# burlachenkok/flpytorch

Hardware: AMD Instinct MI355X
Metric: gradient-codec encode+reduce GB/s (device-resident), [N,D] fp32; % HBM peak (higher is better)
Workload: dtype f32; 1 GPU; C3 topk:1% N=1024/GPU D=10000000; codec=topk:1%, clients_per_gpu=1024, clients_total=1024, D=10000000, K=100000, rows_alloc=contiguous, parallelism=client-shard dp1

## Files before the change

flpytorch_amd/_lib.py:

```python
import collections
import ctypes
import os
import threading

_HERE = os.path.dirname(os.path.abspath(__file__))
VARIANT_DIR = os.path.join(os.path.dirname(_HERE), "abvar")
LIB_PATH = (os.path.join(VARIANT_DIR, "libflcodec_%s.so" % os.environ["FLC_LIB_VARIANT"])
            if os.environ.get("FLC_LIB_VARIANT") else os.path.join(_HERE, "libflcodec.so"))

FLC_OK, FLC_ERR_ARG, FLC_ERR_DTYPE, FLC_ERR_HIP, FLC_ERR_WORKSPACE, FLC_ERR_UNSUPPORTED = range(6)
FLC_IDENT, FLC_LAZY, FLC_RANDK, FLC_NATURAL, FLC_STD_DITHERING, FLC_NAT_DITHERING, FLC_TOPK, FLC_RANK_K = range(1, 9)
FLC_NORM_LINF, FLC_NORM_L1, FLC_NORM_L2 = 0, 1, 2
FLC_REDUCE_PLAIN, FLC_REDUCE_REL_X = 0, 1
FLC_PATH_AUTO, FLC_PATH_SPARSE, FLC_PATH_DENSE = 0, 1, 2
FLC_TIE_LOWEST, FLC_TIE_HIGHEST = 0, 1
FLC_NORMMODE_EXACT, FLC_NORMMODE_TORCH_CPU = 0, 1
ABI_VERSION = 104


def FLC_ROW_GROUPS(g):
    return (int(g) & 0xFF) << 8

EXPORTS = [
    "flc_version", "flc_build_id", "flc_last_error_string",
    "flc_reduce_rows", "flc_reduce_matrix",
    "flc_encode_workspace_size", "flc_encode",
    "flc_encode_reduce_workspace_size", "flc_encode_reduce",
    "flc_encode_reduce_ex_workspace_size", "flc_encode_reduce_ex",
    "flc_encode_shift_workspace_size", "flc_encode_shift",
    "flc_encode_shift_reduce_workspace_size", "flc_encode_shift_reduce",
    "flc_randk_shift_reduce_workspace_size", "flc_randk_shift_reduce",
    "flc_topk_shift_reduce_workspace_size", "flc_topk_shift_reduce",
    "flc_dither_shift_reduce_workspace_size", "flc_dither_shift_reduce", "flc_dither_row_flags",
    "flc_payload_bytes", "flc_payload_format", "flc_payload_validate", "flc_pack_workspace_size", "flc_pack", "flc_unpack",
    "flc_unpack_reduce_workspace_size", "flc_unpack_reduce",
    "flc_pack_shift_workspace_size", "flc_pack_shift",
    "flc_unpack_shift_reduce_workspace_size", "flc_unpack_shift_reduce",
    "flc_combine_workspace_size", "flc_combine_partials",
    "flc_combine_blocks_workspace_size", "flc_combine_blocks",
    "flc_mt_choice", "flc_mt_rand", "flc_mt_randint31",
    "flc_device_uniform", "flc_device_randk_indices",
    "flc_device_randk_counts_workspace_size", "flc_device_randk_counts",
    "flc_profile_enable", "flc_profile_collect", "flc_select_row_flags",
    "flc_selftest_division", "flc_norm2_torch_cpu", "flc_debug_resident",
    "flc_norm2_torch_cpu_workspace_size", "flc_norm2_torch_cpu_ws", "flc_rows_alloc", "flc_rows_free",
]


class FlcCodecParams(ctypes.Structure):
    _fields_ = [
        ("codec", ctypes.c_int32),
        ("s", ctypes.c_int32),
        ("norm", ctypes.c_int32),
        ("flags", ctypes.c_int32),
        ("k", ctypes.c_int64),
        ("lazy_p", ctypes.c_float),
        ("randk_scale", ctypes.c_float),
        ("d_levels", ctypes.c_void_p),
        ("seed", ctypes.c_uint64),
        ("tie", ctypes.c_int32),
    ]


class FlcPattern(ctypes.Structure):
    _fields_ = [
        ("d_randk_idx", ctypes.c_void_p),
        ("d_uniforms", ctypes.c_void_p),
        ("d_lazy_u", ctypes.c_void_p),
        ("client0", ctypes.c_int64),
        ("uniforms_ld", ctypes.c_int64),
        ("idx_ld", ctypes.c_int64),
        ("d_randk_counts", ctypes.c_void_p),
    ]


class FlcShiftRows(ctypes.Structure):
    _fields_ = [
        ("d_a", ctypes.c_void_p), ("lda", ctypes.c_int64),
# ... 127 lines not shown
                                       vp, sz, vp]
        lib.flc_unpack_shift_reduce_workspace_size.argtypes = [P(FlcCodecParams), i64, i64]
        lib.flc_unpack_shift_reduce_workspace_size.restype = sz
        lib.flc_unpack_shift_reduce.argtypes = [P(FlcCodecParams), P(FlcPayloadRows), i64, i64, vp, f32, vp, vp, sz, vp]
    lib.flc_combine_workspace_size.argtypes = [vp, i64, i32]
    lib.flc_combine_workspace_size.restype = sz
    lib.flc_combine_partials.argtypes = [vp, vp, i64, f32, i32, vp, sz, vp]
    lib.flc_combine_blocks_workspace_size.argtypes = [vp, i64, i64]
    lib.flc_combine_blocks_workspace_size.restype = sz
    lib.flc_combine_blocks.argtypes = [vp, vp, i64, i64, i64, f32, vp, vp, sz, vp]
    lib.flc_mt_choice.argtypes = [vp, vp, i64, i64, vp, vp]
    lib.flc_mt_rand.argtypes = [vp, vp, i64, vp]
    lib.flc_mt_randint31.argtypes = [vp, vp, i64, vp]
    lib.flc_device_uniform.argtypes = [ctypes.c_uint64, i64, i64]
    lib.flc_device_uniform.restype = ctypes.c_double
    lib.flc_device_randk_indices.argtypes = [ctypes.c_uint64, i64, i64, i64, vp]
    lib.flc_device_randk_counts_workspace_size.argtypes = [i64, i64]
    lib.flc_device_randk_counts_workspace_size.restype = sz
    lib.flc_device_randk_counts.argtypes = [ctypes.c_uint64, i64, i64, i64, i64, vp, vp, sz, vp]
    lib.flc_profile_enable.argtypes = [i32]
    lib.flc_profile_collect.argtypes = [ctypes.c_char_p, vp, vp]
    lib.flc_selftest_division.argtypes = [vp, i32, vp, vp]
    if hasattr(lib, "flc_norm2_torch_cpu"):
        lib.flc_norm2_torch_cpu.argtypes = [vp, i64, i64, i64, vp, vp]
    if hasattr(lib, "flc_norm2_torch_cpu_ws"):
        lib.flc_norm2_torch_cpu_workspace_size.argtypes = [i64, i64]
        lib.flc_norm2_torch_cpu_workspace_size.restype = sz
        lib.flc_norm2_torch_cpu_ws.argtypes = [vp, i64, i64, i64, vp, vp, sz, vp]
    if hasattr(lib, "flc_rows_alloc"):
        lib.flc_rows_alloc.argtypes = [sz, i32, vp]
        lib.flc_rows_free.argtypes = [vp]
    if hasattr(lib, "flc_debug_resident"):
        lib.flc_debug_resident.argtypes = [i32, i64]
    if hasattr(lib, "flc_select_row_flags"):
        lib.flc_select_row_flags.argtypes = [P(FlcCodecParams), i64, i64, vp, sz, vp, vp]
    for name in EXPORTS:
        if not hasattr(lib, name):
            continue
        if name not in ("flc_version", "flc_build_id", "flc_last_error_string", "flc_device_uniform",
                        "flc_encode_workspace_size", "flc_encode_reduce_workspace_size",
                        "flc_encode_reduce_ex_workspace_size", "flc_encode_shift_workspace_size",
                        "flc_encode_shift_reduce_workspace_size", "flc_randk_shift_reduce_workspace_size",
                        "flc_topk_shift_reduce_workspace_size", "flc_dither_shift_reduce_workspace_size",
                        "flc_payload_bytes", "flc_pack_workspace_size",
                        "flc_pack_shift_workspace_size", "flc_unpack_shift_reduce_workspace_size",
                        "flc_unpack_reduce_workspace_size", "flc_combine_workspace_size",
                        "flc_combine_blocks_workspace_size", "flc_device_randk_counts_workspace_size",
                        "flc_norm2_torch_cpu_workspace_size"):
            getattr(lib, name).restype = i32
    return lib


def source_hash(root=None):
    import glob
    import hashlib
    root = root or os.path.dirname(_HERE)
    csrc = os.path.join(root, "flpytorch_amd", "csrc")
    files = sorted(glob.glob(os.path.join(csrc, "*.hip")) + glob.glob(os.path.join(csrc, "*.hpp")) +
                   glob.glob(os.path.join(csrc, "*.cpp")))
    files += [os.path.join(csrc, "Makefile"), os.path.join(root, "include", "flcodec.h")]
    h = hashlib.sha256()
    for f in files:
        with open(f, "rb") as fh:
            h.update(fh.read())
    return h.hexdigest()[:16]

# ... 89 lines not shown
```

flpytorch_amd/csrc/api.hip:

```cpp
#include <stdarg.h>
#include <stdio.h>

#include <algorithm>
#include <map>
#include <mutex>
#include <string>
#include <vector>

#include "common.hpp"

namespace flc {

static thread_local char g_err[512] = "";

void set_error(const char* fmt, ...) {
    va_list ap;
    va_start(ap, fmt);
    vsnprintf(g_err, sizeof(g_err), fmt, ap);
    va_end(ap);
}

int hip_fail(hipError_t e, const char* what) {
    set_error("%s: %s", what, hipGetErrorString(e));
    return FLC_ERR_HIP;
// ... 155 lines not shown
    if (!d_ptr || bytes == 0) { set_error("flc_rows_alloc: bad args"); return FLC_ERR_ARG; }
    *d_ptr = nullptr;
    const hipError_t e = contiguous ? hipExtMallocWithFlags(d_ptr, bytes, hipDeviceMallocContiguous) : hipMalloc(d_ptr, bytes);
    if (e != hipSuccess) {
        (void)hipGetLastError();
        *d_ptr = nullptr;
        set_error("flc_rows_alloc: %s of %zu bytes failed: %s", contiguous ? "contiguous allocation" : "hipMalloc", bytes,
                  hipGetErrorString(e));
        return FLC_ERR_HIP;
    }
    return FLC_OK;
}

extern "C" int flc_rows_free(void* d_ptr) {
    if (d_ptr && hipFree(d_ptr) != hipSuccess) { set_error("flc_rows_free: hipFree failed"); return FLC_ERR_HIP; }
    return FLC_OK;
}

extern "C" size_t flc_norm2_torch_cpu_workspace_size(int64_t n, int64_t d) {
    return (n <= 0 || d < 0) ? 0 : norm_torch_ws_bytes(n, d);
}

extern "C" int flc_norm2_torch_cpu_ws(const float* d_rows, int64_t ld, int64_t n, int64_t d, float* d_out, void* d_ws,
                                      size_t ws_bytes, void* stream) {
    if (n < 0 || d < 0 || (n > 1 && ld < d) || (n > 0 && (!d_rows || !d_out || !d_ws))) {
        set_error("flc_norm2_torch_cpu_ws: bad args (n=%lld d=%lld ld=%lld)", (long long)n, (long long)d, (long long)ld);
        return FLC_ERR_ARG;
    }
    if (n == 0) return FLC_OK;
    return norm_torch_ws_run(d_rows, ld, n, d, d_out, d_ws, ws_bytes, (hipStream_t)stream);
}

extern "C" int flc_debug_resident(int grid_mult, int64_t spin_ticks) { return rs_debug(grid_mult, spin_ticks); }

extern "C" int flc_norm2_torch_cpu(const float* d_rows, int64_t ld, int64_t n, int64_t d, float* d_out, void* stream) {
    if (n < 0 || d < 0 || (n > 1 && ld < d) || (n > 0 && (!d_rows || !d_out))) {
        set_error("flc_norm2_torch_cpu: bad args (n=%lld d=%lld ld=%lld)", (long long)n, (long long)d, (long long)ld);
        return FLC_ERR_ARG;
    }
    if (n == 0) return FLC_OK;
    return norm_torch_run(d_rows, ld, n, d, d_out, (hipStream_t)stream);
}

namespace flc {
int selftest_division(const float* d_b, int nb, unsigned long long* d_bad, hipStream_t st);
}
extern "C" int flc_selftest_division(const float* d_divisors, int n, unsigned long long* d_mismatches,
                                     void* stream) {
    if (n < 0 || (n > 0 && (!d_divisors || !d_mismatches))) { set_error("flc_selftest_division: bad args"); return FLC_ERR_ARG; }
    if (n == 0) return FLC_OK;
    return selftest_division(d_divisors, n, d_mismatches, (hipStream_t)stream);
}

namespace flc {
size_t encode_row_workspace(const flc_codec_params* prm, int64_t d) {
    if (prm->codec == FLC_TOPK) return sel_workspace(prm, 1, d);
    if (prm->codec == FLC_RANK_K) return rk_workspace(prm, 1, d, false);
    if (prm->codec == FLC_RANDK) return randk_device_workspace(1, d);
    return ew_workspace(prm, 1, d);
}
}

extern "C" size_t flc_encode_workspace_size(const flc_codec_params* prm, int64_t d) {
    if (!prm || !known(prm->codec)) return 0;
    if (prm->codec == FLC_TOPK) return sel_workspace(prm, 1, d);
    if (prm->codec == FLC_RANK_K) return rk_workspace(prm, 1, d, false);
// ... 348 lines not shown
```

flpytorch_amd/csrc/chunk_accum.hip:

```cpp
#include "select_impl.hpp"

namespace flc {

constexpr int AP = FLC_CA_AP;

struct RowMeta {
    uint2 te;
    uint32_t thr, cut, mode;
    float w;
};

__device__ inline RowMeta load_meta(const SelWs& ws, int64_t c, int64_t n, int64_t r, const float* w, int64_t rend = -1) {
    RowMeta m;
    m.te = make_uint2(0, 0);
    m.thr = 0; m.cut = 0u; m.mode = 0; m.w = 1.f;
    if (r < (rend < 0 ? n : rend)) {
        m.te = ws.tab[c * n + r];
        m.thr = ws.thr[r];
        const uint32_t f = ws.flags[r];
        m.mode = (f & F_EXACT) ? 2u : ((f & F_TIES) ? 1u : 0u);
        if (m.mode == 1u) m.cut = tie_pref(ws.tiecut[r], ws.tie_hi);
        if (m.mode == 2u) m.thr = 0u;
        if (w) m.w = w[r];
    }
// ... 81 lines not shown
        if (w && (__float_as_uint(w[r]) >> 31)) continue;
#pragma unroll
        for (int j = 0; j < WL; ++j) if (lane + 64 * j < NW) rm[lane + 64 * j] = 0u;
        __threadfence_block();
        const RowMeta m = load_meta(ws, c, n, r, w);
        const uint32_t mode = m.mode, T = m.thr, cut = m.cut;
        for (uint32_t e = (uint32_t)lane; e < m.te.y; e += 64) {
            const uint32_t ix = ws.ent_idx[r * ws.cap + m.te.x + e];
            const uint32_t key = mag_key(ws.ent_val[r * ws.cap + m.te.x + e]);
            const uint32_t loc = ix - cbase;
            if (loc < (uint32_t)TS && (mode == 2u || key > T || (key == T && tie_pref(ix, ws.tie_hi) >= cut)))
                atomicOr(&rm[loc >> 5], 1u << (loc & 31));
        }
        __threadfence_block();
        bool left = false;
#pragma unroll
        for (int j = 0; j < WL; ++j) {
            if (lane + 64 * j < NW) zc[j] &= atomicOr(&rm[lane + 64 * j], 0u);
            left |= zc[j] != 0u;
        }
        if (__ballot(left) == 0ull) break;
    }
#pragma unroll
    for (int j = 0; j < WL; ++j) {
        uint32_t dead = z0[j] & ~zc[j];
        while (dead) {
            const int b = __builtin_ctz(dead);
            dead &= dead - 1u;
            tl[(lane + 64 * j) * 32 + b] = 0.f;
        }
    }
}

template <bool ASSIGN, int TS, bool W, int WPB, int AP = AP>
__device__ __forceinline__ void chunk_accum_body(int64_t n, int64_t d, SelWs ws, const float* __restrict__ w, float wt,
                                                 float* __restrict__ out, int64_t r0, int64_t rend, int first, int last,
                                                 float (*tile)[TS], uint32_t (*zmask)[WPB == 1 ? 1 : TS / 32]) {
    if (rend < 0) rend = n;
    constexpr int PARTS = CHUNK / TS;
    const int lane = threadIdx.x & 63;
    const int wv = WPB == 1 ? 0 : __builtin_amdgcn_readfirstlane(threadIdx.x >> 6);
    const int64_t C = nchunks(d);
    float* tl = tile[wv];
    const int64_t nb = (rend - r0 + 63) / 64;
    for (int64_t t = (int64_t)blockIdx.x * WPB + wv; t < C * PARTS; t += (int64_t)gridDim.x * WPB) {
        const int64_t c = t / PARTS;
        const uint32_t cbase = (uint32_t)(c * CHUNK + (t % PARTS) * TS);
        if (FLC_TILE_V4 && !ASSIGN && !first && (int64_t)cbase + TS <= d) {
            const float4* p4 = reinterpret_cast<const float4*>(ws.part + cbase);
#pragma unroll
            for (int k0 = 0; k0 < TS / 256; k0 += 8) {
                float4 v[8];
#pragma unroll
                for (int k = 0; k < 8; ++k) v[k] = k0 + k < TS / 256 ? p4[(k0 + k) * 64 + lane] : make_float4(0.f, 0.f, 0.f, 0.f);
#pragma unroll
                for (int k = 0; k < 8; ++k)
                    if (k0 + k < TS / 256) reinterpret_cast<float4*>(tl)[(k0 + k) * 64 + lane] = v[k];
            }
        } else {
            for (int i = lane; i < TS; i += 64)
                tl[i] = ASSIGN ? 0.f : (first || (int64_t)cbase + i >= d ? -0.f : ws.part[cbase + i]);
        }
        RowMeta cur = load_meta(ws, c, n, r0 + lane, w, rend), nxt;
        uint32_t ri[AP][2];
        float rv[AP][2];
        auto fetch = [&](const RowMeta& m, int q, int64_t row, int slot) {
            const uint32_t off = __builtin_amdgcn_readlane(m.te.x, q), cnt = __builtin_amdgcn_readlane(m.te.y, q);
            const auto di = list_rsrc(ws.ent_idx + row * ws.cap + off, cnt);
            const auto dv = list_rsrc(ws.ent_val + row * ws.cap + off, cnt);
#pragma unroll
            for (int h = 0; h < 2; ++h) {
                const uint32_t e = (uint32_t)lane + 64u * h;
                const uint32_t x = __builtin_amdgcn_raw_buffer_load_b32(di, lane * 4, h * 256, 0);
                ri[slot][h] = e < cnt ? x : 0xFFFFFFFFu;
                rv[slot][h] = __uint_as_float(__builtin_amdgcn_raw_buffer_load_b32(dv, lane * 4, h * 256, 0));
            }
        };
        const uint32_t txm = ws.tie_hi ? 0u : 0xFFFFFFFFu;
// ... 62 lines not shown
                    for (int z = 0; z < AP; ++z)
                        if (z == slot) { ri[z][0] = xi[0]; ri[z][1] = xi[1]; rv[z][0] = xv[0]; rv[z][1] = xv[1]; }
                }
            }
            cur = nxt;
        }
        const int64_t len = min((int64_t)TS, d - (int64_t)cbase);
        if (!last) {
            for (int64_t i = lane; i < len; i += 64) ws.part[cbase + i] = tl[i];
            continue;
        }
        if (!ASSIGN) {
            if (WPB == 1) resolve_neg_zero_g<TS>(tl, ws.zm + t * (TS / 32), ws, c, n, cbase, len, w, lane);
            else resolve_neg_zero<TS>(tl, zmask[wv], ws, c, n, cbase, len, w, lane);
        }
        for (int64_t i = lane; i < len; i += 64) out[cbase + i] = ASSIGN ? tl[i] : tl[i] / wt;
    }
}

template <bool ASSIGN, int TS = CHUNK, bool W = true>
__global__ __launch_bounds__(256) void k_chunk_accum(int64_t n, int64_t d, SelWs ws, const float* __restrict__ w, float wt,
                                                     float* __restrict__ out, int64_t r0 = 0, int64_t rend = -1,
                                                     int first = 1, int last = 1) {
    __shared__ __attribute__((aligned(16))) float tile[4][TS];
    __shared__ uint32_t zmask[4][TS / 32];
    chunk_accum_body<ASSIGN, TS, W, 4>(n, d, ws, w, wt, out, r0, rend, first, last, tile, zmask);
}

template <bool W>
__global__ __launch_bounds__(64) void k_chunk_accum1(
        int64_t n, int64_t d, SelWs ws, const float* __restrict__ w, float wt, float* __restrict__ out, int64_t r0,
        int64_t rend, int first, int last) {
    extern __shared__ __attribute__((aligned(16))) float dyn_tile[];
    chunk_accum_body<false, CHUNK, W, 1, FLC_CA_AP1>(n, d, ws, w, wt, out, r0, rend, first, last,
                                         reinterpret_cast<float (*)[CHUNK]>(dyn_tile), nullptr);
}

__global__ __launch_bounds__(256) void k_assign_scatter(SelWs ws, float* __restrict__ out, int sharded) {
    const uint32_t T = ws.thr[0], f = ws.flags[0];
    const uint32_t mode = (f & F_EXACT) ? 2u : ((f & F_TIES) ? 1u : 0u);
    const uint32_t cut = mode == 1u ? tie_pref(ws.tiecut[0], ws.tie_hi) : 0u;
    const bool shd = sharded && mode != 2u;
    const int64_t segcap = (ws.cap / CS_SH) & ~int64_t(3);
    for (int sh = shd ? (int)blockIdx.x : 0; sh < (shd ? CS_SH : 1); sh += shd ? (int)gridDim.x : 1) {
        const uint32_t cnt = shd ? ws.shcnt[sh * RCS] : ws.rowcnt[0];
        const int64_t o = shd ? sh * segcap : 0;
        for (uint32_t e = (shd ? 0u : blockIdx.x * 256u) + threadIdx.x; e < cnt; e += shd ? 256u : gridDim.x * 256u) {
            const uint32_t ix = ws.ent_idx[o + e];
            const float v = ws.ent_val[o + e];
            const uint32_t key = mag_key(v);
            if (mode == 2u || key > T || (key == T && tie_pref(ix, ws.tie_hi) >= cut)) out[ix] = v;
        }
    }
}

static int accum_parts() {
    static const int p = [] {
        const char* e = tuning_env("FLC_ACCUM_PARTS");
        const int v = e ? atoi(e) : 0;
        return (v == 1 || v == 2 || v == 4) ? v : 0;
    }();
    return p;
}

int launch_group_fold(int64_t n, int64_t d, SelWs ws, const float* w, float wt, float* out, int64_t r0, int64_t r1,
                      bool first, bool last, bool exposed, hipStream_t st) {
    const int64_t C = host_chunks(d);
// ... 57 lines not shown
```

flpytorch_amd/csrc/common.hpp:

```cpp
#pragma once
#include <hip/hip_runtime.h>
#include <stdint.h>
#include <stdlib.h>
#include <string.h>

#include "../../include/flcodec.h"

namespace flc {

constexpr int WAVE = 64;
constexpr int CHUNK = 4096;
constexpr int CHUNK_SHIFT = 12;

void set_error(const char* fmt, ...);
int hip_fail(hipError_t e, const char* what);

#define FLC_CHECK_HIP(expr)                                          \
    do {                                                             \
        hipError_t _e = (expr);                                      \
        if (_e != hipSuccess) return ::flc::hip_fail(_e, #expr);     \
    } while (0)
#define FLC_CHECK_LAUNCH(what)                                       \
    do {                                                             \
        hipError_t _e = hipGetLastError();                           \
// ... 129 lines not shown
int shift_epi_launch(const float* e, int64_t d, const ShiftArgs& sh, hipStream_t st);
int shift_fold_launch(const float* m, int64_t d, const float* w, int64_t i, bool last, float wt, float* acc,
                      hipStream_t st);
enum { SHAPE_D = 0, SHAPE_A = 1, SHAPE_C = 2, SHAPE_B = 3 };
int shift_shape(const flc_shift_rows& sr, const char* me);
int inplace_rows_check(const char* me, int shape, const flc_shift_rows& sr, int64_t n, int64_t d);
int sparse_round_precheck(const char* me, int shape, const flc_shift_rows& sr, int64_t n, int64_t d, int64_t K);
int fold_updated_rows(const flc_shift_rows& sr, int64_t n, int64_t d, const float* w, float wt, float* out, hipStream_t st);
int64_t pack_blocks(int64_t d);
int pack_sparse_launch(const float* dense, int64_t d, int64_t cap, uint32_t* bc, char* payload, hipStream_t st);
size_t pack_shift_workspace(const flc_codec_params* prm, int64_t d);
int pack_shift_run(const flc_codec_params* prm, const flc_pattern* pat, const float* a, int64_t d, const ShiftArgs& sh,
                   char* payload, void* ws, size_t ws_bytes, hipStream_t st);
size_t unpack_shift_reduce_workspace(const flc_codec_params* prm, int64_t n, int64_t d);
int unpack_shift_reduce_run(const flc_codec_params* prm, const flc_payload_rows& pr, int64_t n, int64_t d,
                            const float* w, float wt, float* out, void* ws, size_t ws_bytes, hipStream_t st);
inline int64_t group_row(int64_t n, int G, int g, int lastpct) {
    lastpct = lastpct < 1 ? 1 : lastpct;
    if (G <= 1 || lastpct >= 100) return n * g / G;
    const int64_t unit = 100 * (int64_t)(G - 1) + lastpct;
    const int64_t cum = g <= G - 1 ? 100 * (int64_t)g : unit;
    return n * cum / unit;
}
int norm_torch_run(const float* x, int64_t ld, int64_t n, int64_t d, float* out, hipStream_t st);
size_t norm_torch_ws_bytes(int64_t n, int64_t d);
int norm_torch_ws_run(const float* x, int64_t ld, int64_t n, int64_t d, float* out, void* wsp, size_t ws_bytes,
                      hipStream_t st);
int tn_run(RowSrc rows, int64_t n, int64_t r0, int64_t rn, int64_t d, float* out, void* wsp, const double* item_sums,
           int64_t G, hipStream_t st);
size_t sel_workspace(const flc_codec_params* prm, int64_t n, int64_t d);
int sel_run(const flc_codec_params* prm, const flc_pattern* pat, RowSrc rows, bool vec, int64_t n, int64_t d,
            bool assign, const float* w, float wt, float* out, void* wsp, size_t ws_bytes, hipStream_t st);
int rs_debug(int mult, int64_t spin_ticks);
int sel_row_flags(const flc_codec_params* prm, int64_t n, int64_t d, const void* wsp, size_t ws_bytes,
                  uint32_t* flags, hipStream_t st);
bool ds_eligible(const flc_codec_params* prm, const flc_pattern* pat, int64_t n, int64_t d);
size_t ds_workspace(const flc_codec_params* prm, int64_t n, int64_t d, int norm_mode = FLC_NORMMODE_EXACT);
int ds_run(const flc_codec_params* prm, const flc_pattern* pat, RowSrc rows, int64_t n, int64_t d, const float* w,
           float wt, float* pnorm_out, float* out, void* wsp, size_t ws_bytes, hipStream_t st,
           const float* pnorm_in = nullptr, int norm_mode = FLC_NORMMODE_EXACT);
size_t rk_workspace(const flc_codec_params* prm, int64_t n, int64_t d, bool reduce);
int rk_run(const flc_codec_params* prm, RowSrc rows, int64_t n, int64_t d, bool reduce, const float* w, float wt,
           float* out, void* wsp, size_t ws_bytes, hipStream_t st);
size_t randk_device_workspace(int64_t n, int64_t d);
int randk_device_counts(uint64_t seed, int64_t client0, int64_t n, int64_t d, int64_t k, uint32_t* cnt, void* ws,
                        size_t ws_bytes, hipStream_t st);
int randk_device_prepare(const flc_codec_params* prm, const flc_pattern* pat, int64_t n, int64_t d, void* wsp,
                         const uint32_t** cnt, const uint64_t** ckey, hipStream_t st);
struct RkLists {
    const uint2* tab;
    const uint32_t* idx;
    float* val;
    int64_t cap;
};
size_t randk_lists_workspace(int64_t n, int64_t d, int64_t K);
int randk_lists_build(const flc_codec_params* prm, const flc_pattern* pat, RowSrc rows, int64_t n, int64_t d, void* wsp,
                      RkLists* lists, hipStream_t st);
int randk_lists_fold(int64_t n, int64_t d, int64_t K, void* wsp, const float* w, float wt, float* out, hipStream_t st);
size_t randk_shift_workspace(const flc_codec_params* prm, bool compat, int64_t n, int64_t d);
int randk_shift_run(const flc_codec_params* prm, const flc_pattern* pat, const flc_shift_rows& sr, int64_t n, int64_t d,
                    const float* w, float wt, float* out, void* ws, size_t ws_bytes, hipStream_t st);
int randk_shift_lfold_launch(const float* base, int64_t n, int64_t d, RkLists lists, const float* w, float wt, float* out,
                             hipStream_t st);
constexpr uint32_t TK_F_TIES = 4u, TK_F_EXACT = 8u;
struct TkLists {
    const uint2* tab;
// ... 111 lines not shown
```

flpytorch_amd/csrc/select.hip:

```cpp
#include "select_impl.hpp"

namespace flc {

int64_t sel_capacity(int codec, int64_t d, int64_t K) {
    if (codec == FLC_RANDK) return std::max<int64_t>(K, 1);
    int64_t cap = 2 * K + 2 * CHUNK;
    cap = std::min<int64_t>(std::max<int64_t>(cap, 1), std::max<int64_t>(d, 1));
    return (cap + 3) & ~int64_t(3);
}

SelWs carve_sel(void* base, int codec, int64_t n, int64_t d, int64_t K, size_t* bytes) {
    Carver cv(base);
    const int64_t C = std::max<int64_t>(host_chunks(d), 1), nn = std::max<int64_t>(n, 1);
    SelWs s;
    s.tie_hi = 0;
    s.cap = sel_capacity(codec, d, K);
    s.tab = cv.take<uint2>((size_t)C * nn);
    s.ent_idx = cv.take<uint32_t>((size_t)nn * s.cap);
    s.ent_val = cv.take<float>((size_t)nn * s.cap);
    s.rowcnt = cv.take<uint32_t>((size_t)nn * RCS);
    s.flags = cv.take<uint32_t>(nn);
    s.thr = cv.take<uint32_t>(nn);
    s.prefix = cv.take<uint32_t>(nn);
    s.krem = cv.take<uint32_t>(nn);
// ... 74 lines not shown

static int topk_fast_groups(const TkCall& c) {
    const int64_t n = c.n, d = c.d;
    const SelWs& ws = c.ws;
    const hipStream_t st = c.st;
    const bool few = c.few;
    const int TG = few ? 1 : tk_tail_groups(c.prm, n);
    hipStream_t sside = st;
    TkCtx* cx = nullptr;
    std::unique_lock<std::mutex> lk;
    if (TG > 1) {
        int dev = 0;
        FLC_CHECK_HIP(hipGetDevice(&dev));
        lk = std::unique_lock<std::mutex>(g_tk_mu);
        cx = &g_tk_ctx[dev];
        if (!cx->side) {
            int lo = 0, hi = 0;
            FLC_CHECK_HIP(hipDeviceGetStreamPriorityRange(&lo, &hi));
            FLC_CHECK_HIP(hipStreamCreateWithPriority(&cx->side, hipStreamNonBlocking, hi));
        }
        while ((int)cx->ev.size() < TG + 3) {
            hipEvent_t e;
            FLC_CHECK_HIP(hipEventCreateWithFlags(&e, FLC_SYNC_EVENT_FLAGS));
            cx->ev.push_back(e);
        }
        sside = cx->side;
    }
    const bool split = FLC_TK_SPLIT_SAMPLE && TG > 1;
    const int64_t rs1 = split ? group_row(n, TG, 1, FLC_TK_LASTPCT) : n;
    if (split) {
        FLC_CHECK_HIP(hipEventRecord(cx->ev[TG + 1], st));
        FLC_CHECK_HIP(hipStreamWaitEvent(sside, cx->ev[TG + 1], 0));
    }
    launch_sample(c, 0, rs1, st);
    FLC_CHECK_LAUNCH("k_topk_sample");
    if (split) {
        launch_sample(c, rs1, n, sside);
        FLC_CHECK_LAUNCH("k_topk_sample (side)");
        FLC_CHECK_HIP(hipEventRecord(cx->ev[TG + 2], sside));
    }
    for (int g = 0; g < TG; ++g) {
        const int64_t r0 = group_row(n, TG, g, FLC_TK_LASTPCT), rn = group_row(n, TG, g + 1, FLC_TK_LASTPCT) - r0;
        if (split && g == 1) FLC_CHECK_HIP(hipStreamWaitEvent(st, cx->ev[TG + 2], 0));
        { ProfScope _ps("k_topk_filter", st);
        launch_filter_rows(c, r0, rn); }
        FLC_CHECK_LAUNCH("k_topk_filter");
        if (TG > 1) {
            FLC_CHECK_HIP(hipEventRecord(cx->ev[g], st));
            FLC_CHECK_HIP(hipStreamWaitEvent(sside, cx->ev[g], 0));
        }
        { ProfScope _ps("k_cand_select", sside);
        launch_select(c, r0, rn, c.gfold ? g == TG - 1 : (TG > 1 && g == TG - 1), sside); }
        FLC_CHECK_LAUNCH("k_cand_select");
        if (c.gfold) {
            const bool lastg = g == TG - 1;
            if (int rc = launch_group_fold(n, d, ws, c.w, c.wt, c.out, r0, r0 + rn, g == 0, lastg, lastg || TG == 1, sside))
                return rc;
        }
    }
    if (!c.lone_assign && !c.gfold) {
        if (int rc = launch_exact_rows(c, sside)) return rc;
    }
    if (TG > 1) {
        FLC_CHECK_HIP(hipEventRecord(cx->ev[TG], sside));
        FLC_CHECK_HIP(hipStreamWaitEvent(st, cx->ev[TG], 0));
    }
    return FLC_OK;
}

static int topk_dense_k(const TkCall& c) {
// ... 147 lines not shown
```

flpytorch_amd/csrc/select_impl.hpp:

```cpp
#pragma once
#include <stdlib.h>

#include <atomic>
#include <map>
#include <mutex>
#include <type_traits>
#include <vector>

#include "chunks.hpp"
#include "randk_tree.hpp"

namespace flc {

constexpr uint32_t ALL = 0xFFFFFFFFu;
constexpr uint32_t F_OVERFLOW = 1u, F_SHORT = 2u, F_TIES = 4u, F_EXACT = 8u;
constexpr uint32_t F_RESIDENT = 16u;
constexpr uint32_t F_REPAIR = 32u;
constexpr int SMAX = 16384;
constexpr int HBINS = 2048;
constexpr uint32_t TIECAP = HBINS;
constexpr int CS_SH = 64;
constexpr int64_t CS_FEW = 16;
constexpr int CS_ST = 8;
constexpr int CS_LCAP = 2048;
// ... 323 lines not shown
}

struct RkdWs {
    uint32_t* cnt;
    uint64_t* ckey;
};

static inline int64_t host_chunks(int64_t d) { return (d + CHUNK - 1) / CHUNK; }
static inline int grid_stride_blocks(int64_t items, int64_t cap = 4096) {
    return (int)std::max<int64_t>(1, std::min<int64_t>(items, cap));
}
template <class F>
static inline void with_vec(bool vec, F f) {
    if (vec) f(std::true_type{});
    else f(std::false_type{});
}

struct TkCall {
    const flc_codec_params* prm;
    RowSrc rows;
    bool vec;
    int64_t n, d, K;
    bool assign;
    const float* w;
    float wt;
    float* out;
    SelWs ws;
    hipStream_t st;
    bool few, lone_assign, gfold;
};

int64_t sel_capacity(int codec, int64_t d, int64_t K);
SelWs carve_sel(void* base, int codec, int64_t n, int64_t d, int64_t K, size_t* bytes);
void launch_sample(const TkCall& c, int64_t a, int64_t b, hipStream_t sx);
void launch_filter_rows(const TkCall& c, int64_t r0, int64_t rn);
int launch_filter_exact(const TkCall& c);
void launch_select(const TkCall& c, int64_t r0, int64_t rn, bool last_of_many, hipStream_t sx);
int launch_exact_rows(const TkCall& c, hipStream_t sx);
int launch_radix_full(const TkCall& c);
int launch_assign_finish(const TkCall& c);
int lone_resident_launch(RowSrc rows, int64_t d, int64_t K, SelWs ws, float* out, hipStream_t st, bool* took);
int randk_lists_launch(const flc_codec_params* prm, const flc_pattern* pat, RowSrc rows, int64_t n, int64_t d, SelWs ws,
                       hipStream_t st);
int randk_device_run(const flc_codec_params* prm, const flc_pattern* pat, RowSrc rows, int64_t n, int64_t d,
                     const float* w, float wt, float* out, void* wsp, size_t ws_bytes, hipStream_t st);
int launch_chunk_accum(int64_t n, int64_t d, SelWs ws, bool assign, const float* w, float wt, float* out, hipStream_t st);
int launch_group_fold(int64_t n, int64_t d, SelWs ws, const float* w, float wt, float* out, int64_t r0, int64_t r1,
                      bool first, bool last, bool exposed, hipStream_t st);
int launch_chunk_accum_whole(int64_t n, int64_t d, SelWs ws, const float* w, float wt, float* out, hipStream_t st);
void launch_assign_scatter(SelWs ws, float* out, bool few, hipStream_t st);

}
```

flpytorch_amd/csrc/topk_filter.hip:

```cpp
#include "select_impl.hpp"

namespace flc {

template <int NT, bool DUAL>
__global__ __launch_bounds__(NT) void k_topk_sample(RowSrc rows, int64_t n, int64_t d, int64_t K, SelWs ws, int few,
                                                    int64_t r_off) {
    __shared__ uint32_t keys[SMAX];
    __shared__ uint32_t h[HBINS], h2[DUAL ? HBINS : 1];
    __shared__ uint32_t scratch[260], scratch2[DUAL ? 260 : 1];
    const int64_t row = r_off + blockIdx.x;
    if (row >= n) return;
    const float* r = rows.row(row);
    int S;
    if (d <= SMAX) {
        S = (int)d;
        for (int i = threadIdx.x; i < S; i += NT) keys[i] = mag_key(r[i]);
    } else {
        const int P = SMAX / 256;
        S = SMAX;
        constexpr int GR = NT / 256, PU = 32 / GR;
        const int e = threadIdx.x & 255, g0 = threadIdx.x >> 8;
        for (int p0 = 0; p0 < P; p0 += 32) {
            float x[PU];
#pragma unroll
// ... 539 lines not shown
        const char* e = tuning_env("FLC_TK_RB");
        return e ? std::max<int64_t>(1, atoll(e)) : (int64_t)64;
    }();
    ProfScope _pv(FGS == 4 ? "k_topk_filter_g4" : "k_topk_filter_g2", st);
    if constexpr (FGS == 4 && FLC_TK_WG != 0 && FLC_TK_PROBE != 1 && FLC_TK_PROBE != 3) {
        static const bool wg = [] { const char* e = tuning_env("FLC_FILTER_WG"); return !(e && atoi(e) == 0); }();
        if (wg && shards == 1 && !zout) {
            constexpr int NL = FLC_TK_WG_NL;
            const int64_t items = rn * ((nchunks(d) + 4 * NL - 1) / (4 * NL));
            const int gi = (int)std::max<int64_t>(1, std::min<int64_t>(items, 32768));
            static const int64_t rbw = [] {
                const char* e = tuning_env("FLC_TK_RB");
                return e ? std::max<int64_t>(1, atoll(e)) : (int64_t)16;
            }();
            hipLaunchKernelGGL((k_topk_filter_fast_wg<FLC_TK_WG_RING, NL>), dim3(gi), dim3((NL + 1) * 64), 0, st, rows, n, r0,
                               rn, std::min(rbw, std::max<int64_t>(rn, 1)), d, ws);
            return;
        }
    }
    if (zout)
        hipLaunchKernelGGL((k_topk_filter_fast<FLC_TK_RING, FGS, 1>), dim3(gw), dim3(256), 0, st, rows, n, r0, rn,
                           std::min(rb, std::max<int64_t>(rn, 1)), d, ws, shards, zout);
    else
        hipLaunchKernelGGL((k_topk_filter_fast<FLC_TK_RING, FGS>), dim3(gw), dim3(256), 0, st, rows, n, r0, rn,
                           std::min(rb, std::max<int64_t>(rn, 1)), d, ws, shards, (float*)nullptr);
}

void launch_filter_rows(const TkCall& c, int64_t r0, int64_t rn) {
    float* zout = c.lone_assign ? c.out : nullptr;
    if (filter_group() == 2 || c.n * c.d < ((int64_t)64 << 20)) launch_filter<2>(c.rows, c.n, r0, rn, c.d, c.ws, c.st, c.few ? CS_SH : 1, zout);
    else launch_filter<4>(c.rows, c.n, r0, rn, c.d, c.ws, c.st, c.few ? CS_SH : 1, zout);
}

void launch_sample(const TkCall& c, int64_t a, int64_t b, hipStream_t sx) {
    if (b <= a) return;
    ProfScope _ps("k_topk_sample", sx);
    hipLaunchKernelGGL((c.few ? k_topk_sample<1024, true> : k_topk_sample<1024, false>), dim3((unsigned)(b - a)), dim3(1024), 0, sx,
                       c.rows, c.n, c.d, c.K, c.ws, c.few ? 1 : 0, a);
}

int launch_filter_exact(const TkCall& c) {
    const int64_t bpr = (host_chunks(c.d) + 3) / 4;
    const int gb = grid_stride_blocks(c.n * bpr, 8192);
    { ProfScope _ps("k_topk_filter_exact", c.st);
    with_vec(c.vec, [&](auto v) {
        hipLaunchKernelGGL((k_topk_filter<true, decltype(v)::value>), dim3(gb), dim3(256), 0, c.st, c.rows, c.n, c.d, c.ws);
    }); }
    FLC_CHECK_LAUNCH("k_topk_filter(exact)");
    return FLC_OK;
}

}
```

flpytorch_amd/csrc/topk_select.hip:

```cpp
#include "select_impl.hpp"

namespace flc {

__device__ inline float4 cs_ld(const float4* p) {
#if FLC_CS_NT
    typedef float v4f __attribute__((ext_vector_type(4)));
    const v4f v = __builtin_nontemporal_load(reinterpret_cast<const v4f*>(p));
    return make_float4(v.x, v.y, v.z, v.w);
#else
    return *p;
#endif
}
template <int NT>
__device__ void cand_select_row(int64_t row, int64_t K, SelWs ws, uint32_t* h, uint32_t* scratch) {
    {
        if (ws.flags[row]) return;
        const uint32_t cnt = ws.rowcnt[(row) * RCS];
        if (cnt < (uint32_t)K) {
            if (threadIdx.x == 0) ws.flags[row] |= F_SHORT;
            return;
        }
        const uint32_t T = ws.thr[row];
        const uint32_t span = ws.prefix[row] - T;
        int s = 0;
        while (s < 21 && (((uint64_t)span * 4u) >> s) >= (uint64_t)HBINS) ++s;
        const float* vals = ws.ent_val + row * ws.cap;
        const float4* v4 = reinterpret_cast<const float4*>(vals);
        const uint32_t n4 = cnt >> 2;
        uint32_t prefix = 0, krem = (uint32_t)K, last = 0;
        bool first = true, fail = false;
        int sh = s;
        while (true) {
            const int s1 = first ? sh : max(0, sh - 11);
            const uint32_t mask = first ? 0xFFFFFFFFu : ((1u << (sh - s1)) - 1u);
            for (int i = threadIdx.x; i < HBINS; i += NT) h[i] = 0;
            __syncthreads();
            auto add = [&](float x) {
                const uint32_t dk = mag_key(x) - T;
                if (first) atomicAdd(&h[min(dk >> s1, (uint32_t)(HBINS - 1))], 1u);
                else if ((dk >> sh) == prefix) atomicAdd(&h[(dk >> s1) & mask], 1u);
            };
            uint32_t i = threadIdx.x;
            for (; i + 7 * NT < n4; i += 8 * NT) {
                float4 q[8];
#pragma unroll
                for (int u = 0; u < 8; ++u) q[u] = cs_ld(v4 + i + u * NT);
#pragma unroll
                for (int u = 0; u < 8; ++u) { add(q[u].x); add(q[u].y); add(q[u].z); add(q[u].w); }
            }
            for (; i < n4; i += NT) {
                const float4 q = v4[i];
                add(q.x); add(q.y); add(q.z); add(q.w);
            }
            for (uint32_t i = n4 * 4 + threadIdx.x; i < cnt; i += NT) add(vals[i]);
            __syncthreads();
            uint32_t bin, above;
            hist_find(h, krem, bin, above, scratch);
            last = h[bin];
            if (first && bin == HBINS - 1) { fail = true; break; }
            prefix = first ? bin : ((prefix << (sh - s1)) | bin);
            krem -= above;
            sh = s1;
            first = false;
            __syncthreads();
            if (sh == 0) break;
        }
        __syncthreads();
        const uint32_t thr = T + prefix;
        bool ties = !fail && last > krem;
        if (ties && last > TIECAP) { fail = true; ties = false; }
        if (ties) {
            uint32_t* tix = h;
            if (threadIdx.x == 0) scratch[0] = 0;
            __syncthreads();
            const uint32_t* idxs = ws.ent_idx + row * ws.cap;
            for (uint32_t i = threadIdx.x; i < n4; i += NT) {
                const float4 q = v4[i];
                const float qv[4] = {q.x, q.y, q.z, q.w};
#pragma unroll
// ... 415 lines not shown
                erank += eq[q] ? 1u : 0u;
                na += adm[q] ? 1u : 0u;
            }
            uint32_t atot;
            uint32_t pos = base + ex_scan<NT>(na, wsum, atot);
#pragma unroll
            for (int q = 0; q < 4; ++q)
                if (adm[q]) { oi[pos] = (uint32_t)(j0 + q); ov[pos] = v[q]; ++pos; }
            base += atot;
            tie_run += etot;
            if (sb == SUBS - 1 && t == 0) ws.tab[c * n + row] = make_uint2(cbase, base - cbase);
        }
        if (t == 0) {
            ws.thr[row] = thr;
            ws.krem[row] = krem;
            ws.rowcnt[row * RCS] = base;
            ws.flags[row] = F_EXACT | (ws.flags[row] & (F_OVERFLOW | F_SHORT));
        }
        __syncthreads();
    }
}

template <bool VEC>
__global__ __launch_bounds__(EX_NT) void k_topk_exact_rows(RowSrc rows, int64_t n, int64_t r0, int64_t rn, int64_t d, int64_t K, SelWs ws) {
    __shared__ uint32_t h[HBINS];
    __shared__ uint32_t scratch[260];
    __shared__ uint32_t wsum[EX_NT / 64];
    for (int64_t row = r0 + blockIdx.x; row < r0 + rn; row += gridDim.x) {
        if (!(ws.flags[row] & (F_OVERFLOW | F_SHORT))) continue;
        exact_row<VEC>(rows, n, row, d, K, ws, h, scratch, wsum);
    }
}

template <int NT, bool VEC>
__global__ __launch_bounds__(NT) void k_cand_select_x(RowSrc rows, int64_t n, int64_t r0, int64_t rn, int64_t d, int64_t K,
                                                      SelWs ws) {
    __shared__ uint32_t h[HBINS];
    __shared__ uint32_t scratch[260];
    __shared__ uint32_t wsum[NT / 64];
    __shared__ uint32_t failed;
    for (int64_t row = r0 + blockIdx.x; row < r0 + rn; row += gridDim.x) {
        cand_select_row<NT>(row, K, ws, h, scratch);
        __syncthreads();
        if (threadIdx.x == 0) failed = __atomic_load_n(&ws.flags[row], __ATOMIC_RELAXED) & (F_OVERFLOW | F_SHORT);
        __syncthreads();
        if (failed) exact_row<VEC, NT>(rows, n, row, d, K, ws, h, scratch, wsum);
        __syncthreads();
    }
}

__global__ __launch_bounds__(256) void k_tie_count(RowSrc rows, int64_t n, int64_t d, SelWs ws) {
    const int64_t C = nchunks(d);
    const int lane = threadIdx.x & 63, wv = threadIdx.x >> 6;
    const int64_t nrows = *ws.nwork;
    const int64_t bpr = (C + 3) / 4;
    for (int64_t it = blockIdx.x; it < nrows * bpr; it += gridDim.x) {
        const int64_t row = ws.worklist[it / bpr];
        const int64_t c = (it % bpr) * 4 + wv;
        if (c >= C) continue;
        uint32_t cnt = 0;
        if (ws.flags[row] & F_TIES) {
            const uint32_t T = ws.thr[row];
            const float* r = rows.row(row);
            const int64_t j1 = min(d, (c + 1) * (int64_t)CHUNK);
            for (int64_t j = c * CHUNK + lane; j < j1; j += 64) cnt += (mag_key(r[j]) == T) ? 1u : 0u;
            cnt = wave_sum(cnt);
        }
        if (lane == 0) ws.tieprefix[c * n + row] = cnt;
    }
}

__global__ __launch_bounds__(256) void k_tie_scan(int64_t n, int64_t d, SelWs ws) {
    constexpr bool EXACT = true;
    __shared__ uint32_t part[256];
    const int64_t C = nchunks(d);
// ... 22 lines not shown
        }
        __syncthreads();
    }
}

template <bool VEC>
__global__ __launch_bounds__(EX_NT) void k_assign_finish(RowSrc rows, int64_t d, int64_t K, SelWs ws, float* __restrict__ out) {
    __shared__ uint32_t h[HBINS];
    __shared__ uint32_t scratch[260];
    __shared__ uint32_t wsum[EX_NT / 64];
    if (ws.flags[0] & (F_OVERFLOW | F_SHORT)) {
        if (blockIdx.x != 0) return;
        exact_row<VEC>(rows, 1, 0, d, K, ws, h, scratch, wsum);
        __threadfence_block();
        const uint32_t cnt = ws.rowcnt[0];
        for (uint32_t e = threadIdx.x; e < cnt; e += EX_NT) out[ws.ent_idx[e]] = ws.ent_val[e];
        return;
    }
    const uint32_t T = ws.thr[0], f = ws.flags[0];
    const uint32_t cut = (f & F_TIES) ? tie_pref(ws.tiecut[0], ws.tie_hi) : 0u;
    const int64_t segcap = (ws.cap / CS_SH) & ~int64_t(3);
    for (int sh = (int)blockIdx.x; sh < CS_SH; sh += (int)gridDim.x) {
        const uint32_t cnt = ws.shcnt[sh * RCS];
        const int64_t o = sh * segcap;
        for (uint32_t e = threadIdx.x; e < cnt; e += EX_NT) {
            const uint32_t ix = ws.ent_idx[o + e];
            const float v = ws.ent_val[o + e];
            const uint32_t key = mag_key(v);
            if (key > T || (key == T && tie_pref(ix, ws.tie_hi) >= cut)) out[ix] = v;
        }
    }
}

void launch_select(const TkCall& c, int64_t r0, int64_t rn, bool last_of_many, hipStream_t sx) {
    const int64_t n = c.n, d = c.d, K = c.K;
    const SelWs& ws = c.ws;
    if (c.few) {
        const int np = (FLC_CS_LIST && d <= FLC_CS_TWO_MAXD) ? 2 : 3;
        for (int p = 0; p < np; ++p)
            hipLaunchKernelGGL(k_cs_pass, dim3((unsigned)CS_SH, (unsigned)n), dim3(CS_NT), 0, c.st, K, ws,
                               p == np - 1 ? 1 : 0);
    } else if (c.gfold) {
        const bool big = rn < 128 || last_of_many;
        const int nt = big ? 1024 : FLC_TK_SIDE_NT;
        const dim3 grid((unsigned)(big ? rn : grid_stride_blocks(rn, 8192)));
        with_vec(c.vec, [&](auto v) {
            constexpr bool V = decltype(v)::value;
            if (big) hipLaunchKernelGGL((k_cand_select_x<1024, V>), grid, dim3(nt), 0, sx, c.rows, n, r0, rn, d, K, ws);
            else if (FLC_TK_SIDE_NT == 256) hipLaunchKernelGGL((k_cand_select_x<256, V>), grid, dim3(nt), 0, sx, c.rows, n, r0, rn, d, K, ws);
            else hipLaunchKernelGGL((k_cand_select_x<512, V>), grid, dim3(nt), 0, sx, c.rows, n, r0, rn, d, K, ws);
        });
    } else if (rn < 128 || last_of_many)
        hipLaunchKernelGGL(k_cand_select<1024>, dim3((unsigned)rn), dim3(1024), 0, sx, r0, rn, K, ws);
    else if (FLC_TK_SIDE_NT == 256)
        hipLaunchKernelGGL(k_cand_select<256>, dim3(grid_stride_blocks(rn, 8192)), dim3(256), 0, sx, r0, rn, K, ws);
    else hipLaunchKernelGGL(k_cand_select<512>, dim3(grid_stride_blocks(rn, 8192)), dim3(512), 0, sx, r0, rn, K, ws);
}

int launch_exact_rows(const TkCall& c, hipStream_t sx) {
    ProfScope _ps("k_topk_exact_rows", sx);
    const int eb = grid_stride_blocks(c.n, FLC_TK_EXACT_WG);
    with_vec(c.vec, [&](auto v) {
        hipLaunchKernelGGL((k_topk_exact_rows<decltype(v)::value>), dim3(eb), dim3(EX_NT), 0, sx, c.rows, c.n, (int64_t)0, c.n, c.d, c.K, c.ws);
    });
    FLC_CHECK_LAUNCH("k_topk_exact_rows");
    return FLC_OK;
}

int launch_radix_full(const TkCall& c) {
    const int64_t n = c.n, d = c.d, K = c.K;
    const SelWs& ws = c.ws;
    const hipStream_t st = c.st;
    const int64_t bpr = (host_chunks(d) + 3) / 4;
    hipLaunchKernelGGL(k_build_worklist, dim3(1), dim3(1024), 0, st, n, K, d, ws, 1);
    FLC_CHECK_LAUNCH("k_build_worklist");
    const int64_t hb = (d + 65535) / 65536;
    for (int p = 0; p < 3; ++p) {
        { ProfScope _ps("k_radix_hist_full", st);
        hipLaunchKernelGGL((k_radix_hist<true>), dim3(grid_stride_blocks(n * hb)), dim3(256), 0, st, c.rows, n, d, p, ws); }
        FLC_CHECK_LAUNCH("k_radix_hist(full)");
        hipLaunchKernelGGL((k_radix_select<true>), dim3(grid_stride_blocks(n, 1024)), dim3(256), 0, st, n, p, K, ws);
        FLC_CHECK_LAUNCH("k_radix_select(full)");
    }
// ... 18 lines not shown
```

include/flcodec.h:

```cpp
#ifndef FLCODEC_H
#define FLCODEC_H

#include <stddef.h>
#include <stdint.h>

#ifdef __cplusplus
extern "C" {
#endif

typedef enum {
    FLC_OK = 0,
    FLC_ERR_ARG = 1,
    FLC_ERR_DTYPE = 2,
    FLC_ERR_HIP = 3,
    FLC_ERR_WORKSPACE = 4,
    FLC_ERR_UNSUPPORTED = 5
} flc_status;

typedef enum {
    FLC_IDENT = 1,
    FLC_LAZY = 2,
    FLC_RANDK = 3,
    FLC_NATURAL = 4,
    FLC_STD_DITHERING = 5,
// ... 151 lines not shown
int flc_combine_blocks(void* rccl_comm, const float* d_blocks, int64_t ld, int64_t nb_local, int64_t d,
                       float w_total, float* d_out, void* d_ws, size_t ws_bytes, void* stream);

int flc_mt_choice(uint32_t* h_key, int32_t* h_pos, int64_t n, int64_t k, int64_t* h_out,
                  int64_t* h_scratch);
int flc_mt_rand(uint32_t* h_key, int32_t* h_pos, int64_t n, double* h_out);
int flc_mt_randint31(uint32_t* h_key, int32_t* h_pos, int64_t count, int64_t* h_out);

double flc_device_uniform(uint64_t seed, int64_t client, int64_t j);
int flc_device_randk_indices(uint64_t seed, int64_t client, int64_t d, int64_t k, int64_t* h_out);
size_t flc_device_randk_counts_workspace_size(int64_t n, int64_t d);
int flc_device_randk_counts(uint64_t seed, int64_t client0, int64_t n, int64_t d, int64_t k, uint32_t* d_counts,
                            void* d_ws, size_t ws_bytes, void* stream);

int flc_norm2_torch_cpu(const float* d_rows, int64_t ld, int64_t n, int64_t d, float* d_out, void* stream);

size_t flc_norm2_torch_cpu_workspace_size(int64_t n, int64_t d);
int flc_norm2_torch_cpu_ws(const float* d_rows, int64_t ld, int64_t n, int64_t d, float* d_out, void* d_ws,
                           size_t ws_bytes, void* stream);

int flc_selftest_division(const float* d_divisors, int n, unsigned long long* d_mismatches, void* stream);

int flc_profile_enable(int on);
int flc_profile_collect(const char* kernel, double* h_total_ms, int64_t* h_launches);

int flc_select_row_flags(const flc_codec_params* prm, int64_t n, int64_t d, const void* d_workspace,
                         size_t ws_bytes, uint32_t* d_flags, void* stream);

int flc_rows_alloc(size_t bytes, int contiguous, void** d_ptr);
int flc_rows_free(void* d_ptr);

int flc_debug_resident(int grid_mult, int64_t spin_ticks);

#ifdef __cplusplus
}
#endif
#endif
```

Measured before the change: 5967 GB/s.

## Cap side-stream select grid by candidate footprint, XCD-spread chunk accumulation, dual-mode sampling

The side-stream candidate-select grid is now sized so the candidate bytes in flight stay near 32 MB instead of launching up to 8192 blocks, and its first histogram pass uses plain loads in place of streaming cs_ld loads. The single-chunk accumulate kernel remaps block work items round-robin across 8 XCDs. The sample kernel switches to its dual variant when it runs alone with at most one block per CU. A debug hook that overrides the select grid size is also added. These aim to reduce cache thrashing and improve L2 locality, at the cost of possibly less parallelism on the side stream.

```diff
diff --git a/flpytorch_amd/_lib.py b/flpytorch_amd/_lib.py
--- a/flpytorch_amd/_lib.py
+++ b/flpytorch_amd/_lib.py
@@ -44,6 +44,7 @@
     "flc_profile_enable", "flc_profile_collect", "flc_select_row_flags",
     "flc_selftest_division", "flc_norm2_torch_cpu", "flc_debug_resident",
     "flc_norm2_torch_cpu_workspace_size", "flc_norm2_torch_cpu_ws", "flc_rows_alloc", "flc_rows_free",
+    "flc_debug_select_rows",
 ]
 
 
@@ -237,6 +238,8 @@
         lib.flc_rows_free.argtypes = [vp]
     if hasattr(lib, "flc_debug_resident"):
         lib.flc_debug_resident.argtypes = [i32, i64]
+    if hasattr(lib, "flc_debug_select_rows"):
+        lib.flc_debug_select_rows.argtypes = [i32]
     if hasattr(lib, "flc_select_row_flags"):
         lib.flc_select_row_flags.argtypes = [P(FlcCodecParams), i64, i64, vp, sz, vp, vp]
     for name in EXPORTS:
diff --git a/flpytorch_amd/csrc/api.hip b/flpytorch_amd/csrc/api.hip
--- a/flpytorch_amd/csrc/api.hip
+++ b/flpytorch_amd/csrc/api.hip
@@ -211,6 +211,7 @@
 }
 
 extern "C" int flc_debug_resident(int grid_mult, int64_t spin_ticks) { return rs_debug(grid_mult, spin_ticks); }
+extern "C" int flc_debug_select_rows(int rows_in_flight) { return select_rows_debug(rows_in_flight); }
 
 extern "C" int flc_norm2_torch_cpu(const float* d_rows, int64_t ld, int64_t n, int64_t d, float* d_out, void* stream) {
     if (n < 0 || d < 0 || (n > 1 && ld < d) || (n > 0 && (!d_rows || !d_out))) {
diff --git a/flpytorch_amd/csrc/chunk_accum.hip b/flpytorch_amd/csrc/chunk_accum.hip
--- a/flpytorch_amd/csrc/chunk_accum.hip
+++ b/flpytorch_amd/csrc/chunk_accum.hip
@@ -137,7 +137,13 @@
     }
 }
 
-template <bool ASSIGN, int TS, bool W, int WPB, int AP = AP>
+__device__ __forceinline__ int64_t xcd_item(int64_t v, int64_t total) {
+    constexpr int64_t NX = 8;
+    const int64_t q = total / NX, r = total % NX, x = v % NX;
+    return x * q + (x < r ? x : r) + v / NX;
+}
+
+template <bool ASSIGN, int TS, bool W, int WPB, int AP = AP, bool XCD = false>
 __device__ __forceinline__ void chunk_accum_body(int64_t n, int64_t d, SelWs ws, const float* __restrict__ w, float wt,
                                                  float* __restrict__ out, int64_t r0, int64_t rend, int first, int last,
                                                  float (*tile)[TS], uint32_t (*zmask)[WPB == 1 ? 1 : TS / 32]) {
@@ -148,7 +154,10 @@
     const int64_t C = nchunks(d);
     float* tl = tile[wv];
     const int64_t nb = (rend - r0 + 63) / 64;
-    for (int64_t t = (int64_t)blockIdx.x * WPB + wv; t < C * PARTS; t += (int64_t)gridDim.x * WPB) {
+    const int64_t items = (C * PARTS + WPB - 1) / WPB;
+    for (int64_t v = blockIdx.x; v < items; v += gridDim.x) {
+        const int64_t t = (XCD ? xcd_item(v, items) : v) * WPB + wv;
+        if (t >= C * PARTS) continue;
         const int64_t c = t / PARTS;
         const uint32_t cbase = (uint32_t)(c * CHUNK + (t % PARTS) * TS);
         if (FLC_TILE_V4 && !ASSIGN && !first && (int64_t)cbase + TS <= d) {
@@ -277,7 +286,7 @@
         int64_t n, int64_t d, SelWs ws, const float* __restrict__ w, float wt, float* __restrict__ out, int64_t r0,
         int64_t rend, int first, int last) {
     extern __shared__ __attribute__((aligned(16))) float dyn_tile[];
-    chunk_accum_body<false, CHUNK, W, 1, FLC_CA_AP1>(n, d, ws, w, wt, out, r0, rend, first, last,
+    chunk_accum_body<false, CHUNK, W, 1, FLC_CA_AP1, true>(n, d, ws, w, wt, out, r0, rend, first, last,
                                          reinterpret_cast<float (*)[CHUNK]>(dyn_tile), nullptr);
 }
 
diff --git a/flpytorch_amd/csrc/common.hpp b/flpytorch_amd/csrc/common.hpp
--- a/flpytorch_amd/csrc/common.hpp
+++ b/flpytorch_amd/csrc/common.hpp
@@ -185,6 +185,7 @@
 int sel_run(const flc_codec_params* prm, const flc_pattern* pat, RowSrc rows, bool vec, int64_t n, int64_t d,
             bool assign, const float* w, float wt, float* out, void* wsp, size_t ws_bytes, hipStream_t st);
 int rs_debug(int mult, int64_t spin_ticks);
+int select_rows_debug(int rows_in_flight);
 int sel_row_flags(const flc_codec_params* prm, int64_t n, int64_t d, const void* wsp, size_t ws_bytes,
                   uint32_t* flags, hipStream_t st);
 bool ds_eligible(const flc_codec_params* prm, const flc_pattern* pat, int64_t n, int64_t d);
diff --git a/flpytorch_amd/csrc/select.hip b/flpytorch_amd/csrc/select.hip
--- a/flpytorch_amd/csrc/select.hip
+++ b/flpytorch_amd/csrc/select.hip
@@ -130,10 +130,10 @@
         FLC_CHECK_HIP(hipEventRecord(cx->ev[TG + 1], st));
         FLC_CHECK_HIP(hipStreamWaitEvent(sside, cx->ev[TG + 1], 0));
     }
-    launch_sample(c, 0, rs1, st);
+    launch_sample(c, 0, rs1, split, st);
     FLC_CHECK_LAUNCH("k_topk_sample");
     if (split) {
-        launch_sample(c, rs1, n, sside);
+        launch_sample(c, rs1, n, false, sside);
         FLC_CHECK_LAUNCH("k_topk_sample (side)");
         FLC_CHECK_HIP(hipEventRecord(cx->ev[TG + 2], sside));
     }
diff --git a/flpytorch_amd/csrc/select_impl.hpp b/flpytorch_amd/csrc/select_impl.hpp
--- a/flpytorch_amd/csrc/select_impl.hpp
+++ b/flpytorch_amd/csrc/select_impl.hpp
@@ -379,7 +379,7 @@
 
 int64_t sel_capacity(int codec, int64_t d, int64_t K);
 SelWs carve_sel(void* base, int codec, int64_t n, int64_t d, int64_t K, size_t* bytes);
-void launch_sample(const TkCall& c, int64_t a, int64_t b, hipStream_t sx);
+void launch_sample(const TkCall& c, int64_t a, int64_t b, bool alone, hipStream_t sx);
 void launch_filter_rows(const TkCall& c, int64_t r0, int64_t rn);
 int launch_filter_exact(const TkCall& c);
 void launch_select(const TkCall& c, int64_t r0, int64_t rn, bool last_of_many, hipStream_t sx);
diff --git a/flpytorch_amd/csrc/topk_filter.hip b/flpytorch_amd/csrc/topk_filter.hip
--- a/flpytorch_amd/csrc/topk_filter.hip
+++ b/flpytorch_amd/csrc/topk_filter.hip
@@ -595,10 +595,21 @@
     else launch_filter<4>(c.rows, c.n, r0, rn, c.d, c.ws, c.st, c.few ? CS_SH : 1, zout);
 }
 
-void launch_sample(const TkCall& c, int64_t a, int64_t b, hipStream_t sx) {
+static int chip_cus() {
+    static const int v = [] {
+        int dev = 0, cus = 0;
+        if (hipGetDevice(&dev) != hipSuccess ||
+            hipDeviceGetAttribute(&cus, hipDeviceAttributeMultiprocessorCount, dev) != hipSuccess) return 0;
+        return cus;
+    }();
+    return v;
+}
+
+void launch_sample(const TkCall& c, int64_t a, int64_t b, bool alone, hipStream_t sx) {
     if (b <= a) return;
     ProfScope _ps("k_topk_sample", sx);
-    hipLaunchKernelGGL((c.few ? k_topk_sample<1024, true> : k_topk_sample<1024, false>), dim3((unsigned)(b - a)), dim3(1024), 0, sx,
+    const bool dual = c.few || (alone && b - a <= chip_cus());
+    hipLaunchKernelGGL((dual ? k_topk_sample<1024, true> : k_topk_sample<1024, false>), dim3((unsigned)(b - a)), dim3(1024), 0, sx,
                        c.rows, c.n, c.d, c.K, c.ws, c.few ? 1 : 0, a);
 }
 
diff --git a/flpytorch_amd/csrc/topk_select.hip b/flpytorch_amd/csrc/topk_select.hip
--- a/flpytorch_amd/csrc/topk_select.hip
+++ b/flpytorch_amd/csrc/topk_select.hip
@@ -11,7 +11,7 @@
     return *p;
 #endif
 }
-template <int NT>
+template <int NT, bool SIDE = false>
 __device__ void cand_select_row(int64_t row, int64_t K, SelWs ws, uint32_t* h, uint32_t* scratch) {
     {
         if (ws.flags[row]) return;
@@ -40,11 +40,17 @@
                 if (first) atomicAdd(&h[min(dk >> s1, (uint32_t)(HBINS - 1))], 1u);
                 else if ((dk >> sh) == prefix) atomicAdd(&h[(dk >> s1) & mask], 1u);
             };
+            const bool plain = SIDE && first;
             uint32_t i = threadIdx.x;
             for (; i + 7 * NT < n4; i += 8 * NT) {
                 float4 q[8];
-#pragma unroll
-                for (int u = 0; u < 8; ++u) q[u] = cs_ld(v4 + i + u * NT);
+                if (plain) {
+#pragma unroll
+                    for (int u = 0; u < 8; ++u) q[u] = v4[i + u * NT];
+                } else {
+#pragma unroll
+                    for (int u = 0; u < 8; ++u) q[u] = cs_ld(v4 + i + u * NT);
+                }
 #pragma unroll
                 for (int u = 0; u < 8; ++u) { add(q[u].x); add(q[u].y); add(q[u].z); add(q[u].w); }
             }
@@ -526,7 +532,7 @@
     }
 }
 
-template <int NT, bool VEC>
+template <int NT, bool VEC, bool SIDE = false>
 __global__ __launch_bounds__(NT) void k_cand_select_x(RowSrc rows, int64_t n, int64_t r0, int64_t rn, int64_t d, int64_t K,
                                                       SelWs ws) {
     __shared__ uint32_t h[HBINS];
@@ -534,7 +540,7 @@
     __shared__ uint32_t wsum[NT / 64];
     __shared__ uint32_t failed;
     for (int64_t row = r0 + blockIdx.x; row < r0 + rn; row += gridDim.x) {
-        cand_select_row<NT>(row, K, ws, h, scratch);
+        cand_select_row<NT, SIDE>(row, K, ws, h, scratch);
         __syncthreads();
         if (threadIdx.x == 0) failed = __atomic_load_n(&ws.flags[row], __ATOMIC_RELAXED) & (F_OVERFLOW | F_SHORT);
         __syncthreads();
@@ -623,6 +629,14 @@
     }
 }
 
+constexpr int64_t SIDE_SELECT_BYTES = int64_t(32) << 20;
+static std::atomic<int> g_select_rows{0};
+int select_rows_debug(int rows_in_flight) {
+    if (rows_in_flight < 0) { set_error("flc_debug_select_rows: rows in flight >= 0"); return FLC_ERR_ARG; }
+    g_select_rows.store(rows_in_flight, std::memory_order_relaxed);
+    return FLC_OK;
+}
+
 void launch_select(const TkCall& c, int64_t r0, int64_t rn, bool last_of_many, hipStream_t sx) {
     const int64_t n = c.n, d = c.d, K = c.K;
     const SelWs& ws = c.ws;
@@ -634,12 +648,20 @@
     } else if (c.gfold) {
         const bool big = rn < 128 || last_of_many;
         const int nt = big ? 1024 : FLC_TK_SIDE_NT;
-        const dim3 grid((unsigned)(big ? rn : grid_stride_blocks(rn, 8192)));
+        int64_t rf = rn;
+        if (!big) {
+            const double ks = std::max(1.0, (double)K * (double)std::min<int64_t>(d, SMAX) / (double)d);
+            const double row_bytes = 4.0 * (double)K * (1.0 + 4.0 / sqrt(ks));
+            rf = (int64_t)ceil((double)SIDE_SELECT_BYTES / row_bytes);
+        }
+        const int dbg = g_select_rows.load(std::memory_order_relaxed);
+        if (dbg > 0) rf = dbg;
+        const dim3 grid((unsigned)std::max<int64_t>(1, std::min<int64_t>(rf, std::min<int64_t>(rn, 8192))));
         with_vec(c.vec, [&](auto v) {
             constexpr bool V = decltype(v)::value;
             if (big) hipLaunchKernelGGL((k_cand_select_x<1024, V>), grid, dim3(nt), 0, sx, c.rows, n, r0, rn, d, K, ws);
-            else if (FLC_TK_SIDE_NT == 256) hipLaunchKernelGGL((k_cand_select_x<256, V>), grid, dim3(nt), 0, sx, c.rows, n, r0, rn, d, K, ws);
-            else hipLaunchKernelGGL((k_cand_select_x<512, V>), grid, dim3(nt), 0, sx, c.rows, n, r0, rn, d, K, ws);
+            else if (FLC_TK_SIDE_NT == 256) hipLaunchKernelGGL((k_cand_select_x<256, V, true>), grid, dim3(nt), 0, sx, c.rows, n, r0, rn, d, K, ws);
+            else hipLaunchKernelGGL((k_cand_select_x<512, V, true>), grid, dim3(nt), 0, sx, c.rows, n, r0, rn, d, K, ws);
         });
     } else if (rn < 128 || last_of_many)
         hipLaunchKernelGGL(k_cand_select<1024>, dim3((unsigned)rn), dim3(1024), 0, sx, r0, rn, K, ws);
diff --git a/include/flcodec.h b/include/flcodec.h
--- a/include/flcodec.h
+++ b/include/flcodec.h
@@ -207,6 +207,8 @@
 
 int flc_debug_resident(int grid_mult, int64_t spin_ticks);
 
+int flc_debug_select_rows(int rows_in_flight);
+
 #ifdef __cplusplus
 }
 #endif
```

Result: no change. 5957 GB/s (-0.2%).
